# gcorso/DiffDock

Hardware: NVIDIA H100
Metric: poses/sec at 20 diffusion steps (higher is better)
Workload: dtype f32

## Files before the change

### diffdock_b200/cg_model.py

```python
from __future__ import annotations

import math
import os

import numpy as np
import torch
from torch import nn

from . import ops
from .irreps import irreps_str, sh_irreps
from .hetero import receptor_blocks
from .layers import (AtomEncoder, GaussianSmearing, _mlp, check_confidence_widths, check_forward, confidence_head, cross_cutoff,
                     cross_graph, edge_cutoff, edge_weight, ligand_graph, score_heads)
from .synthetic import LIG_FEATURE_DIMS as lig_feature_dims, REC_RESIDUE_FEATURE_DIMS as rec_residue_feature_dims
from .tensor_layers import TensorProductConvLayer, get_irrep_seq
from .tp_table import full_tensor_product

_TABLES = os.path.join(os.path.dirname(os.path.abspath(__file__)), 'tables', 'score_norm_tables.npz')
SO3_MIN_EPS, SO3_MAX_EPS, SO3_N_EPS = 0.0005, 4, 2000
TORUS_SIGMA_MIN, TORUS_SIGMA_MAX, TORUS_SIGMA_N = 3e-3, 2, 5000


def _i32(t):
    return t.to(torch.int32).contiguous()


def _flat(w):
    return w.reshape(-1).contiguous() if torch.is_tensor(w) else None


def _rr_joint(c, n_lig):
    if n_lig not in c.setdefault('rr_tgt32', {}):
        c['rr_tgt32'][n_lig] = (_i32(c['rr_tgt'] + n_lig), _i32(c['rr_src'] + n_lig))
    return c['rr_tgt32'][n_lig]


def receptor_tiles(rec, B, ei):
    blocks = receptor_blocks(rec, B, ei.shape[1])
    if blocks is None:
        return None
    dev = ei.device
    ar = lambda a, b: torch.arange(a, b, device=dev)
# ... 51 lines not shown
        self.scale_by_sigma, self.norm_by_sigma = scale_by_sigma, norm_by_sigma
        self.no_torsion, self.smooth_edges, self.odd_parity = no_torsion, smooth_edges, odd_parity
        self.confidence_mode, self.affinity_prediction = confidence_mode, affinity_prediction
        self.atom_confidence, self.atom_num_confidence_outputs = atom_confidence, atom_num_confidence_outputs
        self.num_conv_layers, self.num_prot_emb_layers = num_conv_layers, num_prot_emb_layers
        self.fixed_center_conv, self.no_aminoacid_identities = fixed_center_conv, no_aminoacid_identities
        self.differentiate_convolutions, self.reduce_pseudoscalars = differentiate_convolutions, reduce_pseudoscalars
        self.embed_also_ligand = embed_also_ligand
        self.lm_embedding_type = lm_embedding_type
        lm_dim = 1280 if lm_embedding_type == 'precomputed' else 0
        S, D, Dx = sigma_embed_dim, distance_embed_dim, cross_distance_embed_dim

        self.lig_node_embedding = AtomEncoder(emb_dim=ns, feature_dims=lig_feature_dims, sigma_embed_dim=S)
        self.lig_edge_embedding = _mlp(in_lig_edge_features + S + D, ns, ns, dropout)
        self.rec_node_embedding = AtomEncoder(emb_dim=ns, feature_dims=rec_residue_feature_dims, sigma_embed_dim=0,
                                              lm_embedding_dim=lm_dim)
        self.rec_edge_embedding = _mlp(D, ns, ns, dropout)
        self.rec_sigma_embedding = _mlp(S, ns, ns, dropout)
        self.cross_edge_embedding = _mlp(S + Dx, ns, ns, dropout)
        self.lig_distance_expansion = GaussianSmearing(0.0, lig_max_radius, D)
        self.rec_distance_expansion = GaussianSmearing(0.0, rec_max_radius, D)
        self.cross_distance_expansion = GaussianSmearing(0.0, cross_max_distance, Dx)

        self._irrep_seq = get_irrep_seq(ns, nv, use_second_order_repr, reduce_pseudoscalars)
        self._conv_kw = dict(sh_irreps=self.sh_irreps, n_edge_features=3 * ns, hidden_features=3 * ns, residual=True,
                             batch_norm=batch_norm, dropout=dropout, faster=sh_lmax == 1 and not use_second_order_repr,
                             tp_weights_layers=tp_weights_layers)
        self.rec_emb_layers = nn.ModuleList([self.conv(i, 1) for i in range(num_prot_emb_layers)])
        if embed_also_ligand:
            self.lig_emb_layers = nn.ModuleList([self.conv(i, 1) for i in range(num_prot_emb_layers)])
        self.conv_layers = self._interaction_stack(4, 2)
        self._sync_free = None
        self._prune_receptor = True
        if confidence_mode:
            self._confidence_heads(confidence_dropout, confidence_no_batchnorm, num_confidence_outputs)
            return

        self.center_distance_expansion = GaussianSmearing(0.0, center_max_distance, D)
        self.center_edge_embedding = _mlp(D + S, ns, ns, dropout)
        self.final_conv = TensorProductConvLayer(in_irreps=self.conv_layers[-1].out_irreps, sh_irreps=self.sh_irreps,
                                                 out_irreps='2x1o + 2x1e' if not odd_parity else '1x1o + 1x1e',
                                                 n_edge_features=2 * ns, residual=False, dropout=dropout,
                                                 batch_norm=batch_norm)
        self.tr_final_layer = nn.Sequential(nn.Linear(1 + S, ns), nn.Dropout(dropout), nn.ReLU(), nn.Linear(ns, 1))
        self.rot_final_layer = nn.Sequential(nn.Linear(1 + S, ns), nn.Dropout(dropout), nn.ReLU(), nn.Linear(ns, 1))
        if not no_torsion:
            self.final_edge_embedding = _mlp(D, ns, ns, dropout)
            T, tor_sh = full_tensor_product(self.sh_irreps, '1x2e')
            self.register_buffer('_tor_tp', torch.from_numpy(T).float(), persistent=False)
            self.tor_bond_conv = TensorProductConvLayer(in_irreps=self.conv_layers[-1].out_irreps,
                                                        sh_irreps=irreps_str(tor_sh),
                                                        out_irreps=f'{ns}x0o + {ns}x0e' if not odd_parity else f'{ns}x0o',
                                                        n_edge_features=3 * ns, residual=False, dropout=dropout,
                                                        batch_norm=batch_norm)
            self.tor_final_layer = nn.Sequential(nn.Linear(2 * ns if not odd_parity else ns, ns, bias=False), nn.Tanh(),
                                                 nn.Dropout(dropout), nn.Linear(ns, 1, bias=False))
        z = np.load(_TABLES)
        self.register_buffer('_so3_table', torch.from_numpy(z['so3_exp_score_norms']).float(), persistent=False)
        self.register_buffer('_torus_table', torch.from_numpy(z['torus_score_norm']).float(), persistent=False)

    def _confidence_heads(self, dropout, no_batchnorm, num_confidence_outputs):
        ns = self.ns
        self._conf_tail = (self.nv if self.reduce_pseudoscalars else ns) \
            if self.num_conv_layers + self.num_prot_emb_layers >= 3 else 0
        n_in = ns + self._conf_tail

# ... 78 lines not shown
        c['rr_ew'] = ew[order].contiguous() if torch.is_tensor(ew) else None
        c['rr_tgt_batch'] = rec.batch[tgt]
        c['rec_ptr'] = ops.segment_ptr(rec.batch, B)
        c['lig_ptr'] = ops.segment_ptr(lig.batch, B)
        mask = lig.edge_mask
        bonds = ll.edge_index[:, mask].long()
        c['bonds'], c['n_bonds'] = bonds, int(bonds.shape[1])
        c['bond_batch'] = lig.batch[bonds[0]] if bonds.shape[1] else None
        self._static_sync_free(data, c)
        rr._b200 = c
        return c

    def _static_sync_free(self, data, c):
        rec, lig, ll = data['receptor'], data['ligand'], data['ligand', 'ligand']
        B, dev = data.num_graphs, lig.pos.device
        n_lig, n_rec = lig.batch.shape[0], rec.batch.shape[0]
        lig_cnt = (c['lig_ptr'][1:] - c['lig_ptr'][:-1])
        rec_cnt = (c['rec_ptr'][1:] - c['rec_ptr'][:-1])
        host = torch.stack([lig_cnt, rec_cnt]).cpu()
        c['lig_cnt_f'] = lig_cnt.float().unsqueeze(1)
        c['rec_max'] = int(host[1].max()) if B else 0
        c['cap_cross'] = int((host[0].long() * host[1].long()).sum())
        c['lig_batch32'], c['rec_batch32'] = _i32(lig.batch), _i32(rec.batch)
        c['rr_gid32'] = _i32(c['rr_tgt_batch'])
        ei = ll.edge_index.long()
        order = torch.sort(ei[0], stable=True).indices
        c['pre_tgt'], c['pre_col'] = _i32(ei[0][order]), _i32(ei[1][order])
        attr = ll.edge_attr.float()[order] if ei.shape[1] else torch.zeros((0, self.in_lig_edge_features), device=dev)
        c['pre_attr'] = torch.cat([attr, torch.zeros((1, attr.shape[1]), device=dev)], 0)
        c['cap_ll'] = int(ei.shape[1]) + 33 * n_lig
        c['bond_lig_batch'] = lig.batch[c['bonds'][0]] if c['n_bonds'] else None
        c['cap_tor'] = 32 * c['n_bonds']
        c['bond_batch32'] = _i32(c['bond_batch']) if c['n_bonds'] else None

    def _ligand_graph(self, data, c):
        tgt, src, attr, vec, ew, node = ligand_graph(self, data, c['lig_ptr'])
        tgt, order = torch.sort(tgt, stable=True)
        return node, tgt, src[order], attr[order], vec[order], ew[order] if torch.is_tensor(ew) else ew

    def sync_free_capable(self):
        if self._sync_free is None:
            ok = os.environ.get('DDB200_SYNC_FREE', '1') != '0'
            ok = ok and self.embed_also_ligand
            for layer in list(self.conv_layers) + list(getattr(self, 'lig_emb_layers', [])):
                ok = ok and layer.fused_capable(self.ns, self.ns)
            self._sync_free = bool(ok)
        return self._sync_free

    def sync_free_crop_capable(self):
        return self.sync_free_capable() and all(layer.fused_capable(self.ns, self.ns) for layer in self.rec_emb_layers)

    @torch.no_grad()
    def forward(self, data):
        check_forward(self, data)
        c = self._static(data)
        if self.sync_free_capable() and max(c['rec_max'], c.get('atom_max', 0)) <= 10000:
            return self._forward_sync_free(data, c)
        if getattr(data, '_crop', None) is not None:
            raise RuntimeError("per-step receptor cropping (data._crop) runs on the sync-free forward only, which this "
                               "batch cannot take (more than 10000 residues in a complex)")
        return self._forward_host_sized(data, c)

    def _interaction_layers(self, node, groups, n_last, merge=False, shared=None, per_layer=None):
        L = len(self.conv_layers)
        for l, layer in enumerate(self.conv_layers):
            use, init = (groups if l < L - 1 else groups[:n_last]), None
# ... 1 lines not shown
                k = per_layer[0]
                use = use[:k] + [per_layer[1][l]] + use[k + 1:]
            if l == 0 and shared is not None:
                init, skip = shared
                use = use[:skip] + [None] + use[skip + 1:]
            if merge:
                use = [tuple(torch.cat([g[k] for g in use]) if use[0][k] is not None else None for k in range(5))]
            node = layer.forward_groups(node, use, gather_scalars=self.ns, init=init)
        return node

    def _forward_sync_free(self, data, c):
        lig, rec = data['ligand'], data['receptor']
        ns, n_lig = self.ns, lig.batch.shape[0]
        tr_sigma, rot_sigma, tor_sigma = self._sigmas(data)

        sig = self.rec_sigma_embedding(self.timestep_emb_func(data.complex_t['tr'])).contiguous()
        crop = getattr(data, '_crop', None)
        prune = self._prune_receptor and len(self.conv_layers) > 1
        keep = None
        if crop is None:
            rec_node, rec_pos = rec.rec_node_attr.clone(), rec.pos.float().contiguous()
            rr_tgt32 = _rr_joint(c, n_lig)
            g_rr = (rr_tgt32[0], rr_tgt32[1], c['rr_ea'], c['rr_vec'], _flat(c['rr_ew']),
                    dict(ea_add=sig, ea_add_idx=c['rr_gid32']))
        else:
            rec_node, rec_pos, g_rr, keep = self._cropped_receptor(data, c, crop, sig, n_lig, select=not prune)
        rec_node[:, :ns] += sig[rec.batch]
        lig_node, g_ll = self._ligand_graph_sync_free(data, c)

        r, rpg = cross_cutoff(self, tr_sigma)
        g_lr, g_rl = self._cross_graph_sync_free(data, c, rec_pos, c['rec_ptr'], c['rec_batch32'],
                                                 c['rec_max'], c['cap_cross'], r, rpg, n_lig, self.cross_edge_embedding,
                                                 self.cross_distance_expansion, vec_sign=-1.0)

        node = torch.cat([lig_node, rec_node], 0)
        groups = [g_ll,
                  g_lr,
                  g_rr,
                  g_rl]
        shared = self._shared_receptor_messages(data, c, rec, rec_node, sig, n_lig) \
            if len(self.conv_layers) > 1 and crop is None else None
        pruned = self._pruned_contact_groups(c, g_rl, keep, sig, n_lig, rec_node.shape[0], shared is not None) \
            if prune else None
        node = self._interaction_layers(node, groups, 2, shared=(shared, 2) if shared is not None else None,
                                        per_layer=(2, pruned) if pruned is not None else None)
        return self._heads(data, c, node[:n_lig], tr_sigma, rot_sigma, tor_sigma, sync_free=True)

    def _need_levels(self, L, shared):
        return [None if l == L - 1 or (l == 0 and shared) else L - 1 - l for l in range(L)]

    def _pruned_contact_groups(self, c, g_rl, keep, sig, n_lig, n_rec, shared):
        levels = self._need_levels(len(self.conv_layers), shared)
        n_levels = max((k for k in levels if k is not None), default=0)
        if n_levels == 0:
            return None
        if 'rr_tgt32l' not in c:
            c['rr_tgt32l'] = (_i32(c['rr_tgt']), _i32(c['rr_src']))
        tgt32, src32 = c['rr_tgt32l']
        key = ('prune', n_lig, n_levels)
        if key not in c:
            c[key] = (torch.empty((n_levels, n_rec), dtype=torch.uint8, device=tgt32.device),
                      [ops.select_edges_buffers(tgt32.shape[0], tgt32.device) for _ in range(n_levels)])
        need_buf, bufs = c[key]
        need = ops.receptor_need(g_rl[0], g_rl[5]['n_edges_dev'], n_lig, tgt32, src32, n_rec, n_levels, keep=keep,
                                 out=need_buf)
        ew, sel = _flat(c['rr_ew']), {}
# ... 175 lines not shown
```

### diffdock_b200/csrc/fused_conv.cu

```cuda
#include <cuda_bf16.h>
#include <cuda_runtime.h>
#include <stdint.h>
#include <stdlib.h>

#include "../../include/diffdock_b200.h"
#include "sm90.cuh"

namespace {

using namespace ddb200_sm90;

constexpr int BM = 64, BK = 64;
constexpr int CTA_EDGES = 2 * BM;
constexpr int A_KB_BYTES = BM * BK * 2;
constexpr int B_IMAGE_BYTES = 256 * BK * 2;
constexpr int MAX_N = 192;
constexpr int STAGES = 4;
constexpr int STAGE_BYTES = MAX_N * BK * 2;
constexpr int MAX_KB = 5;
constexpr int MAX_KA = MAX_KB;
constexpr int A_IMAGE_BYTES = MAX_KA * A_KB_BYTES;
constexpr int OPS_PER_KB = 8;
constexpr int THREADS = 256;
constexpr int MAX_TILES = 128, MAX_PATHS = 16, MTAB = 48;
// ... 702 lines not shown
struct DeviceState {
  bool attr_done = false, attr_done_so = false;
  bool dbg_init = false;
  unsigned long long* dbg = nullptr;
};
DeviceState g_dev[MAX_DEVICES];

unsigned long long* fused_debug_buffer(int dev) {
  if (dev < 0 || dev >= MAX_DEVICES) return nullptr;
  DeviceState& st = g_dev[dev];
  if (!st.dbg_init) {
    st.dbg_init = true;
    const char* e = getenv("DDB200_FUSED_DEBUG");
    if (e && atoi(e) != 0 && cudaMalloc(&st.dbg, 32 * sizeof(unsigned long long)) == cudaSuccess)
      cudaMemset(st.dbg, 0, 32 * sizeof(unsigned long long));
  }
  return st.dbg;
}

}


extern "C" int ddb200_fused_debug_read(uint64_t* out) {
  int dev = 0;
  cudaGetDevice(&dev);
  unsigned long long* b = fused_debug_buffer(dev);
  if (!b || !out) return DDB200_EINVAL;
  cudaError_t e = cudaDeviceSynchronize();
  if (e == cudaSuccess) e = cudaMemcpy(out, b, 32 * sizeof(unsigned long long), cudaMemcpyDeviceToHost);
  if (e == cudaSuccess) e = cudaMemset(b, 0, 32 * sizeof(unsigned long long));
  return (int)e;
}

namespace {

template <bool SO>
int fused_conv_launch(const ddb200_fused_args* a, void* stream) {
  if (!a || !a->edge_attr || !a->w1_images || !a->w2_images || !a->tiles || !a->mtab || !a->x || !a->edge_vec || !a->sum ||
      !a->tgt || !a->src || a->n_edges < 0 || a->ne <= 0 || a->ns < 0 || a->hidden <= 0 || a->n_tiles <= 0 || a->d_out <= 0)
    return DDB200_EINVAL;
  if (a->ns > 0 && (!a->node || a->ld_node < a->ns)) return DDB200_EINVAL;
  if (a->n_tiles > MAX_TILES || a->n_paths <= 0 || a->n_paths > (SO ? SO_MAX_PATHS : MAX_PATHS) || a->sh_lmax < 0 ||
      a->sh_lmax > 2)
    return DDB200_EINVAL;
  if ((a->ea_add == nullptr) != (a->ea_add_idx == nullptr)) return DDB200_EINVAL;
  const int K1 = a->ne + 2 * a->ns, H = a->hidden;
  const int K1p = (K1 + 15) / 16 * 16, Hp = (H + 15) / 16 * 16;
  const int n_kb = (2 * Hp + 16 + BK - 1) / BK, n_kb1 = (2 * K1p + 16 + BK - 1) / BK;
  if (n_kb > MAX_KB || n_kb1 > MAX_KB || H > MAX_N) return DDB200_EINVAL;
  if ((reinterpret_cast<uintptr_t>(a->w1_images) & 127) || (reinterpret_cast<uintptr_t>(a->w2_images) & 127)) return DDB200_EINVAL;
  if (a->n_hidden < 0 || (a->n_hidden > 0 && (!a->wh_images || (reinterpret_cast<uintptr_t>(a->wh_images) & 127))))
    return DDB200_EINVAL;
  if (a->n_edges == 0) return 0;
  FusedParams p = {};
  p.ea = a->edge_attr; p.ld_ea = a->ld_ea; p.ne = a->ne; p.node = a->node; p.ld_node = a->ld_node; p.ns = a->ns;
  p.tgt = a->tgt; p.src = a->src; p.perm = a->edge_perm; p.ea_add = a->ea_add; p.ea_add_idx = a->ea_add_idx;
  const auto al16 = [](const void* q) { return (reinterpret_cast<uintptr_t>(q) & 15) == 0; };
  p.a0_vec = ((a->ne | a->ns) & 7) == 0 && ((a->ld_ea | (a->ns ? a->ld_node : 0)) & 3) == 0 && al16(a->edge_attr) &&
             (a->ns == 0 || al16(a->node)) && (a->ea_add == nullptr || al16(a->ea_add));
  p.vec_sign = a->vec_sign == 0.f ? 1.f : a->vec_sign;
  p.w1img = reinterpret_cast<const __nv_bfloat16*>(a->w1_images); p.K1 = K1; p.K1p = K1p; p.n_kb1 = n_kb1;
  p.H = H; p.Hp = Hp; p.n_kb = n_kb;
  p.w2img = reinterpret_cast<const __nv_bfloat16*>(a->w2_images); p.tiles = a->tiles; p.n_tiles = a->n_tiles;
  p.whimg = reinterpret_cast<const __nv_bfloat16*>(a->wh_images); p.n_hidden = a->n_hidden;
  p.mtab = a->mtab; p.n_paths = a->n_paths;
  p.x = a->x; p.ld_x = a->ld_x; p.x_vec2 = (a->x_pairs_ok && (a->ld_x & 1) == 0 && (reinterpret_cast<uintptr_t>(a->x) & 7) == 0) ? 1 : 0;
  p.vec = a->edge_vec; p.ew = a->edge_weight; p.lmax = a->sh_lmax; p.sum = a->sum; p.d_out = a->d_out; p.cnt = a->cnt;
  p.n_edges = a->n_edges; p.n_edges_dev = a->n_edges_dev;
  int dev = 0, sms = 132;
  cudaGetDevice(&dev);
  if (dev < 0 || dev >= MAX_DEVICES) return DDB200_EINVAL;
  p.dbg = fused_debug_buffer(dev);
  cudaDeviceGetAttribute(&sms, cudaDevAttrMultiProcessorCount, dev);
  const long long n_mtiles = (a->n_edges + CTA_EDGES - 1) / CTA_EDGES;
  const size_t smem = smem_bytes<SO>();
  if (smem > 227 * 1024) return DDB200_ESMEM;
  auto kernel = SO ? fused_conv_kernel_so : fused_conv_kernel;
  bool& attr_done = SO ? g_dev[dev].attr_done_so : g_dev[dev].attr_done;
  if (!attr_done) {
    const cudaError_t e = cudaFuncSetAttribute(kernel, cudaFuncAttributeMaxDynamicSharedMemorySize, (int)smem);
    if (e != cudaSuccess) return (int)e;
    attr_done = true;
  }
  const unsigned grid = (unsigned)(n_mtiles < sms ? n_mtiles : sms);
  kernel<<<grid, THREADS, smem, (cudaStream_t)stream>>>(p);
  return (int)cudaGetLastError();
}

}

extern "C" int ddb200_fused_conv(const ddb200_fused_args* a, void* stream) { return fused_conv_launch<false>(a, stream); }

extern "C" int ddb200_fused_conv_so(const ddb200_fused_args* a, void* stream) { return fused_conv_launch<true>(a, stream); }
```

### diffdock_b200/fused.py

```python
from __future__ import annotations

import ctypes as C
import os

import numpy as np
import torch

from . import _lib
from .ops import PROFILE, _need_cuda, _ptr, _stream

from .irreps import real_cg
from .radial import BK, BN
from .tp_table import TpTable

CONSUMER_KINDS = {(48, 1): (0, 4), (10, 3): (1, 16), (16, 1): (2, 8), (4, 3): (3, 16), (10, 1): (4, 16), (4, 1): (5, 16),
                  (10, 5): (6, 16), (4, 5): (7, 16)}
MAX_K = 144
MAX_TILES = 128
MTAB = 48
MAX_PATHS = 16
MTAB_SO = 128
MAX_PATHS_SO = 32
ENABLED = os.environ.get('DDB200_FUSED_CONV', '1') != '0'


def _pad16(k: int) -> int:
    return (k + 15) // 16 * 16


def second_order(table: TpTable) -> bool:
    return any(p.l_in == 2 or p.l_out == 2 for p in table.paths)


def supported(table: TpTable, hidden: int, k1: int) -> bool:
    if table.sh_lmax < 0 or table.sh_lmax > 2:
        return False
    if _pad16(hidden) > MAX_K or _pad16(k1) > MAX_K:
        return False
    if len(table.paths) > (MAX_PATHS_SO if second_order(table) else MAX_PATHS):
        return False
    for p in table.paths:
        if (p.mul_out, 2 * p.l_out + 1) not in CONSUMER_KINDS:
            return False
        if (2 * p.l_in + 1) not in (1, 3, 5) or p.l_sh > 2:
            return False
    n_tiles = sum(-(-p.mul_in // CONSUMER_KINDS[(p.mul_out, 2 * p.l_out + 1)][1]) for p in table.paths)
    return n_tiles <= MAX_TILES


def _split_images(w_rows: torch.Tensor, bias_rows: torch.Tensor, K: int):
    T = w_rows.shape[0]
    Kp = _pad16(K)
    n_kb = (2 * Kp + 16 + BK - 1) // BK
    dev = w_rows.device
    hi = w_rows.to(torch.bfloat16)
# ... 49 lines not shown
                src[:nrow * p.mul_out] = cols
                row_src.append(src)
        for i in range(len(tiles)):
            if i == len(tiles) - 1 or tiles[i + 1][6] & 1:
                tiles[i][6] |= 2
        self.n_tiles = len(tiles)
        self.n_paths = len(paths)
        src = torch.as_tensor(np.stack(row_src), device=dev)
        ok = src >= 0
        w_rows = torch.zeros((self.n_tiles, BN, H), dtype=torch.float32, device=dev)
        b_rows = torch.zeros((self.n_tiles, BN), dtype=torch.float32, device=dev)
        w_rows[ok] = w2_ref.detach().float()[src[ok]]
        b_rows[ok] = b2_ref.detach().float()[src[ok]]
        self.w2_images = _split_images(w_rows, b_rows, H)
        w1p = torch.zeros((1, BN, K1), dtype=torch.float32, device=dev)
        b1p = torch.zeros((1, BN), dtype=torch.float32, device=dev)
        w1p[0, :H], b1p[0, :H] = w1.detach().float(), b1.detach().float()
        self.w1_images = _split_images(w1p, b1p, K1)
        self.wh_images = None
        if hidden:
            whp = torch.zeros((self.n_hidden, BN, H), dtype=torch.float32, device=dev)
            bhp = torch.zeros((self.n_hidden, BN), dtype=torch.float32, device=dev)
            for l, (w, b) in enumerate(hidden):
                whp[l, :H], bhp[l, :H] = w.detach().float(), b.detach().float()
            self.wh_images = _split_images(whp, bhp, H)
        self.tiles = torch.as_tensor(np.asarray(tiles, dtype=np.int32), device=dev).contiguous()
        self.mtab = torch.as_tensor(mtab, device=dev).contiguous()
        self.x_pairs_ok = int(all(t[2] % 2 == 0 and (t[3] * t[4]) % 2 == 0 for t in tiles))
        s2, s1 = 3 * (_pad16(H) // 16) + 1, 3 * (_pad16(K1) // 16) + 1
        self.mma_flops_per_tile = 2 * 64 * 16 * 192 * (s1 + (self.n_hidden + len(tiles)) * s2)
        self.alg_flops_per_edge = 2 * K1 * H + self.n_hidden * 2 * H * H + 2 * H * table.weight_numel + sum(
            2 * p.mul_in * p.mul_out * (2 * p.l_out + 1) + 2 * p.mul_in * (2 * p.l_in + 1) * (2 * p.l_sh + 1) * (2 * p.l_out + 1)
            for p in table.paths)


class _Args(C.Structure):
    _fields_ = [('edge_attr', C.c_void_p), ('ld_ea', C.c_int64), ('ne', C.c_int32),
                ('node', C.c_void_p), ('ld_node', C.c_int64), ('ns', C.c_int32),
                ('tgt', C.c_void_p), ('src', C.c_void_p), ('edge_perm', C.c_void_p),
                ('ea_add', C.c_void_p), ('ea_add_idx', C.c_void_p), ('vec_sign', C.c_float),
                ('w1_images', C.c_void_p), ('hidden', C.c_int32), ('w2_images', C.c_void_p),
                ('tiles', C.c_void_p), ('n_tiles', C.c_int32), ('mtab', C.c_void_p), ('n_paths', C.c_int32),
                ('x', C.c_void_p), ('ld_x', C.c_int64), ('x_pairs_ok', C.c_int32),
                ('edge_vec', C.c_void_p), ('edge_weight', C.c_void_p), ('sh_lmax', C.c_int32),
                ('n_edges', C.c_int64), ('n_edges_dev', C.c_void_p),
                ('sum', C.c_void_p), ('d_out', C.c_int32), ('cnt', C.c_void_p),
                ('wh_images', C.c_void_p), ('n_hidden', C.c_int32)]


def _p(t):
    return t.data_ptr() if t is not None else None


def fused_conv(plan: FusedPlan, edge_attr, node, ns, tgt32, src32, x, edge_vec, sum_buf, cnt_buf, edge_weight=None,
               edge_perm=None, vec_sign=1.0, ea_add=None, ea_add_idx=None, n_edges_dev=None, n_edges=None):
    _need_cuda(edge_attr, x, edge_vec, sum_buf)
    ne = edge_attr.shape[1]
    E = int(tgt32.shape[0]) if n_edges is None else int(n_edges)
    if E == 0:
        return
    t = plan.table
    assert edge_attr.dtype == torch.float32 and edge_attr.stride(1) == 1 and x.stride(1) == 1 and edge_vec.is_contiguous()
    assert edge_vec.dtype == torch.float32 and x.dtype == torch.float32 and sum_buf.dtype == torch.float32
    assert tgt32.dtype == torch.int32 and src32.dtype == torch.int32 and tgt32.is_contiguous() and src32.is_contiguous()
    assert ne + 2 * ns == plan.k1 and x.shape[1] == t.d_in and sum_buf.shape[1] == t.d_out and sum_buf.is_contiguous()
    if edge_perm is None:
        assert edge_attr.shape[0] >= E and edge_vec.shape[0] >= E
    else:
        assert edge_perm.dtype == torch.int32 and edge_perm.is_contiguous() and edge_perm.shape[0] >= E
    if edge_weight is not None:
        edge_weight = edge_weight.reshape(-1)
        assert edge_weight.dtype == torch.float32 and edge_weight.is_contiguous()
    if ea_add is not None:
        assert ea_add.dtype == torch.float32 and ea_add.is_contiguous() and ea_add.shape[1] == ne
        assert ea_add_idx.dtype == torch.int32 and ea_add_idx.is_contiguous() and ea_add_idx.shape[0] >= E
    if n_edges_dev is not None:
        assert n_edges_dev.dtype == torch.int32 and n_edges_dev.is_cuda
    a = _Args(_p(edge_attr), edge_attr.stride(0), ne, _p(node) if ns else None, node.stride(0) if ns else 0, ns,
              _p(tgt32), _p(src32), _p(edge_perm), _p(ea_add), _p(ea_add_idx) if ea_add is not None else None,
              float(vec_sign), _p(plan.w1_images), plan.hidden, _p(plan.w2_images), _p(plan.tiles), plan.n_tiles,
              _p(plan.mtab), plan.n_paths, _p(x), x.stride(0), plan.x_pairs_ok, _p(edge_vec), _p(edge_weight),
              t.sh_lmax, E, _p(n_edges_dev), _p(sum_buf), t.d_out, _p(cnt_buf), _p(plan.wh_images), plan.n_hidden)
    prof = PROFILE.enabled
    if prof:
        e0, e1 = torch.cuda.Event(enable_timing=True), torch.cuda.Event(enable_timing=True)
        e0.record()
    launch = _lib.lib().ddb200_fused_conv_so if plan.second_order else _lib.lib().ddb200_fused_conv
    rc = launch(C.byref(a), _stream())
    if prof:
        e1.record()
        n_live = int(n_edges_dev.item()) if n_edges_dev is not None else E
        PROFILE.fused_pairs.append((e0, e1))
        PROFILE.fused_bytes += n_live * (4 * t.weight_numel + 12 + 4) + 4 * (sum_buf.shape[0] + 1) + \
            4 * x.shape[0] * t.d_in + 4 * sum_buf.shape[0] * t.d_out
        PROFILE.fused_flops += ((n_live + 63) // 64) * plan.mma_flops_per_tile
        PROFILE.fused_alg_flops += n_live * plan.alg_flops_per_edge
    PROFILE.all_launches += 1
    _lib.check(rc, 'ddb200_fused_conv')
```

### include/diffdock_b200.h

```cpp
#ifndef DIFFDOCK_B200_H
#define DIFFDOCK_B200_H

#include <stddef.h>
#include <stdint.h>

#ifdef __cplusplus
extern "C" {
#endif

#define DDB200_EINVAL (-1)
#define DDB200_ETABLE (-2)
#define DDB200_ESMEM  (-3)

const char* ddb200_version(void);

typedef struct ddb200_tp_table ddb200_tp_table;

int  ddb200_tp_table_create(const int32_t* iblob_host, int n_ints, const float* fblob_host, int n_floats,
                            ddb200_tp_table** out);
void ddb200_tp_table_destroy(ddb200_tp_table* t);
int  ddb200_tp_table_info(const ddb200_tp_table* t, int what);

int ddb200_tpconv_accumulate(const ddb200_tp_table* t, const float* x, int64_t x_stride, const int32_t* edge_src,
                             const int32_t* edge_dst, const float* geo, const float* edge_weight, const float* w,
// ... 36 lines not shown

int ddb200_csr_sort_by_target(const int32_t* tgt, int64_t n_edges, int32_t n_rows, int32_t* tgt_sorted, int32_t* perm,
                              int32_t* row_ptr, void* workspace, size_t* workspace_bytes, void* stream);

int ddb200_edge_embed(const float* edge_vec, const int32_t* edge_row, const float* u, const float* w1_rbf, const float* w2,
                      const float* b2, int rbf_dim, int ns, const float* rbf_offset, float rbf_coeff, int64_t capacity,
                      const int32_t* n_edges_dev, float* out, void* stream);

int ddb200_radial_gemm(const float* h, int64_t ldh, int64_t n_edges, int K, const void* b_images, const float* bias,
                       int n_tiles_n, float* out, int64_t ldo, void* stream);

int ddb200_radial_mlp(const float* edge_attr, int64_t ld_ea, int ne, const float* node, int64_t ld_node, int ns,
                      const int32_t* tgt, const int32_t* src, const void* w1_images, const float* b1, int hidden,
                      const void* w2_images, const float* b2, int n_tiles_n, int64_t n_edges, float* out, int64_t ldo,
                      void* stream);

typedef struct ddb200_fused_args {
  const float*   edge_attr;   int64_t ld_ea;   int32_t ne;
  const float*   node;        int64_t ld_node; int32_t ns;
  const int32_t* tgt;         const int32_t* src;
  const int32_t* edge_perm;
  const float*   ea_add;      const int32_t* ea_add_idx;
  float          vec_sign;
  const void*    w1_images;   int32_t hidden;
  const void*    w2_images;
  const int32_t* tiles;       int32_t n_tiles;
  const float*   mtab;        int32_t n_paths;
  const float*   x;           int64_t ld_x;    int32_t x_pairs_ok;
  const float*   edge_vec;    const float* edge_weight;
  int32_t        sh_lmax;
  int64_t        n_edges;     const int32_t* n_edges_dev;
  float*         sum;         int32_t d_out;   float* cnt;
  const void*    wh_images;   int32_t n_hidden;
} ddb200_fused_args;

int ddb200_fused_conv(const ddb200_fused_args* args, void* stream);
int ddb200_fused_conv_so(const ddb200_fused_args* args, void* stream);

int ddb200_fused_debug_read(uint64_t* out);

int ddb200_contact_count(const float* pos, int32_t n, float cutoff, int32_t max_neighbors, int32_t knn_only,
                         int32_t* count, void* stream);
int ddb200_contact_fill(const float* pos, int32_t n, float cutoff, int32_t max_neighbors, int32_t knn_only,
                        const int32_t* row_start, int32_t* out_nbr, int32_t* out_ctr, void* stream);

int ddb200_crop_flags(const float* lig_pos, const int32_t* lig_ptr, const float* rec_pos, const int32_t* rec_batch,
                      int64_t n_rec, const float* cutoff2_table, const int32_t* step_dev, uint8_t* keep,
                      float* rec_pos_masked, void* stream);
int ddb200_crop_select_edges(const int32_t* tgt, const int32_t* src, const int32_t* gid, int64_t n_edges,
                             const uint8_t* keep, const uint8_t* need, int32_t offset, int32_t* out_tgt, int32_t* out_src,
                             int32_t* out_perm, int32_t* out_gid, int32_t* n_selected, void* workspace,
                             size_t* workspace_bytes, void* stream);
int ddb200_receptor_need(const int32_t* cross_tgt, const int32_t* n_cross, int64_t cross_cap, int32_t offset,
                         const int32_t* tgt, const int32_t* src, int64_t n_edges, const uint8_t* keep, int64_t n_rec,
                         int32_t n_levels, uint8_t* need, void* stream);

#define DDB200_CONF_MAX_IN 256
#define DDB200_CONF_MAX_HIDDEN 128
#define DDB200_CONF_MAX_OUT 16
int ddb200_confidence_head(const float* x, int64_t ld_x, int64_t n_cols, const int32_t* lig_ptr, int32_t n_poses,
                           int32_t n_head, int32_t tail_off, int32_t n_tail, const float* atom_mlp, int32_t atom_hidden,
                           int32_t n_atom_out, const float* mlp, int32_t n_in, int32_t n_hidden, int32_t n_out,
                           float* confidence, float* atom_confidence, void* stream);

#ifdef __cplusplus
}
// ... 3 lines not shown
```

Baseline: 23.78.

## Add per-target reassociated tensor-product sum for dense ligand-receptor cross edges

```diff
diff --git a/diffdock_b200/cg_model.py b/diffdock_b200/cg_model.py
--- a/diffdock_b200/cg_model.py
+++ b/diffdock_b200/cg_model.py
@@ -7,7 +7,7 @@
 import torch
 from torch import nn
 
-from . import ops
+from . import fused, ops
 from .irreps import irreps_str, sh_irreps
 from .hetero import receptor_blocks
 from .layers import (AtomEncoder, GaussianSmearing, _mlp, check_confidence_widths, check_forward, confidence_head, cross_cutoff,
@@ -125,6 +125,7 @@
         self.conv_layers = self._interaction_stack(4, 2)
         self._sync_free = None
         self._prune_receptor = True
+        self._ligand_target_sum = True
         if confidence_mode:
             self._confidence_heads(confidence_dropout, confidence_no_batchnorm, num_confidence_outputs)
             return
@@ -269,6 +270,24 @@
         c['bond_lig_batch'] = lig.batch[c['bonds'][0]] if c['n_bonds'] else None
         c['cap_tor'] = 32 * c['n_bonds']
         c['bond_batch32'] = _i32(c['bond_batch']) if c['n_bonds'] else None
+        if getattr(self, '_ligand_target_sum', False):
+            c['lr_target_sum'] = self._ligand_target_sum_workspace(c['cap_cross'], n_lig, dev)
+
+    def _ligand_receptor_plans(self):
+        plans = []
+        for layer in self.conv_layers:
+            fc = layer.fc if layer.edge_groups == 1 else list(layer.fc)[1]
+            plans.append(layer._fused_plan(fc, layer.tp.table_vec, 3 * self.ns) if layer.tp.vec_capable else None)
+        return plans
+
+    def _ligand_target_sum_workspace(self, cap_cross, n_lig, dev):
+        if not (type(self)._forward_sync_free is CGModel._forward_sync_free and not self.confidence_mode
+                and self.sync_free_capable() and cap_cross > 0):
+            return None
+        plans = self._ligand_receptor_plans()
+        if any(p is None or not p.per_target_ok for p in plans):
+            return None
+        return fused.TargetSumWorkspace(cap_cross, n_lig, plans[0].hidden, max(p.ts_zp for p in plans), dev)
 
     def _ligand_graph(self, data, c):
         tgt, src, attr, vec, ew, node = ligand_graph(self, data, c['lig_ptr'])
@@ -336,6 +355,11 @@
         g_lr, g_rl = self._cross_graph_sync_free(data, c, rec_pos, c['rec_ptr'], c['rec_batch32'],
                                                  c['rec_max'], c['cap_cross'], r, rpg, n_lig, self.cross_edge_embedding,
                                                  self.cross_distance_expansion, vec_sign=-1.0)
+        if self._ligand_target_sum:
+            if 'lr_target_sum' not in c:
+                c['lr_target_sum'] = self._ligand_target_sum_workspace(c['cap_cross'], n_lig, lig.pos.device)
+            if c['lr_target_sum'] is not None:
+                g_lr[5]['per_target'] = c['lr_target_sum']
 
         node = torch.cat([lig_node, rec_node], 0)
         groups = [g_ll,
diff --git a/diffdock_b200/csrc/fused_conv.cu b/diffdock_b200/csrc/fused_conv.cu
--- a/diffdock_b200/csrc/fused_conv.cu
+++ b/diffdock_b200/csrc/fused_conv.cu
@@ -758,6 +758,8 @@
   return (int)e;
 }
 
+int target_sum_launch(const ddb200_fused_args* a, void* stream);
+
 namespace {
 
 template <bool SO>
@@ -777,7 +779,12 @@
   if ((reinterpret_cast<uintptr_t>(a->w1_images) & 127) || (reinterpret_cast<uintptr_t>(a->w2_images) & 127)) return DDB200_EINVAL;
   if (a->n_hidden < 0 || (a->n_hidden > 0 && (!a->wh_images || (reinterpret_cast<uintptr_t>(a->wh_images) & 127))))
     return DDB200_EINVAL;
+  if (a->per_target && SO) return DDB200_EINVAL;
   if (a->n_edges == 0) return 0;
+  if (a->per_target) {
+    const int rc = target_sum_launch(a, stream);
+    if (rc) return rc;
+  }
   FusedParams p = {};
   p.ea = a->edge_attr; p.ld_ea = a->ld_ea; p.ne = a->ne; p.node = a->node; p.ld_node = a->ld_node; p.ns = a->ns;
   p.tgt = a->tgt; p.src = a->src; p.perm = a->edge_perm; p.ea_add = a->ea_add; p.ea_add_idx = a->ea_add_idx;
@@ -792,7 +799,7 @@
   p.mtab = a->mtab; p.n_paths = a->n_paths;
   p.x = a->x; p.ld_x = a->ld_x; p.x_vec2 = (a->x_pairs_ok && (a->ld_x & 1) == 0 && (reinterpret_cast<uintptr_t>(a->x) & 7) == 0) ? 1 : 0;
   p.vec = a->edge_vec; p.ew = a->edge_weight; p.lmax = a->sh_lmax; p.sum = a->sum; p.d_out = a->d_out; p.cnt = a->cnt;
-  p.n_edges = a->n_edges; p.n_edges_dev = a->n_edges_dev;
+  p.n_edges = a->n_edges; p.n_edges_dev = a->per_target ? a->ts_sel + 1 : a->n_edges_dev;
   int dev = 0, sms = 132;
   cudaGetDevice(&dev);
   if (dev < 0 || dev >= MAX_DEVICES) return DDB200_EINVAL;
diff --git a/diffdock_b200/csrc/target_sum.cu b/diffdock_b200/csrc/target_sum.cu
--- /dev/null
+++ b/diffdock_b200/csrc/target_sum.cu
@@ -0,0 +1,344 @@
+#include <cuda_runtime.h>
+#include <stdint.h>
+
+#include "../../include/diffdock_b200.h"
+
+namespace {
+
+constexpr int TS_THREADS = 256;
+constexpr int HP = 144;
+constexpr int A_THREADS = 512, A_EDGES = 128, A_LD = A_EDGES + 4;
+constexpr int ZC = 128, CE = 32, HR = 160;
+constexpr int C_TARGETS = 4, C_JSPLIT = 29;
+
+struct TsParams {
+  const float* ea; long long ld_ea; int ne;
+  const float* node; long long ld_node; int ns;
+  const int* tgt; const int* src; const int* perm;
+  const float* ea_add; const int* ea_add_idx;
+  float vec_sign;
+  const float* x; long long ld_x;
+  const float* vec; const float* ew;
+  const float* mtab;
+  float* sum; int d_out; float* cnt;
+  long long n_edges; const int* n_edges_dev;
+  int K1, H;
+  float* hid; int ld;
+  float* S; long long n_targets; int zp;
+  const float* w1t; const float* b1; const float* w2bt; int w2_ld;
+  const int* cols; const int* paths; const int* items; int n_items;
+  int* sel; long long min_edges;
+};
+
+__device__ __forceinline__ long long live_edges(const TsParams& p) {
+  long long n = p.n_edges;
+  if (p.n_edges_dev) { const long long nd = __ldg(p.n_edges_dev); n = nd < n ? (nd < 0 ? 0 : nd) : n; }
+  return n;
+}
+
+__device__ __forceinline__ long long lower_bound(const int* tgt, long long n, int a) {
+  long long lo = 0, hi = n;
+  while (lo < hi) {
+    const long long mid = (lo + hi) >> 1;
+    if (__ldg(tgt + mid) < a) lo = mid + 1; else hi = mid;
+  }
+  return lo;
+}
+
+__device__ __forceinline__ void red_add(float* addr, float v) {
+  asm volatile("red.global.add.f32 [%0], %1;" ::"l"(addr), "f"(v) : "memory");
+}
+
+__global__ void target_sum_select_kernel(const TsParams p) {
+  const long long n = live_edges(p);
+  const int on = n >= p.min_edges;
+  p.sel[0] = on;
+  p.sel[1] = on ? 0 : (int)n;
+}
+
+__global__ void __launch_bounds__(A_THREADS) target_sum_hidden_kernel(const TsParams p) {
+  extern __shared__ __align__(16) float smem[];
+  if (!__ldg(p.sel)) return;
+  float* w1t = smem;
+  float* b1 = w1t + p.K1 * HP;
+  float* aT = b1 + HP;
+  const int tid = threadIdx.x;
+  for (int i = tid; i < p.K1 * HP; i += A_THREADS) w1t[i] = __ldg(p.w1t + i);
+  for (int i = tid; i < HP; i += A_THREADS) b1[i] = __ldg(p.b1 + i);
+  const long long n = live_edges(p);
+  const int eg = tid >> 4, hg = tid & 15;
+  for (long long e0 = (long long)blockIdx.x * A_EDGES; e0 < n; e0 += (long long)gridDim.x * A_EDGES) {
+    __syncthreads();
+    for (int i = tid; i < A_EDGES * p.K1; i += A_THREADS) {
+      const int r = i / p.K1, k = i - r * p.K1;
+      const long long e = e0 + r;
+      float v = 0.f;
+      if (e < n) {
+        if (k < p.ne) {
+          const long long er = p.perm ? (long long)__ldg(p.perm + e) : e;
+          v = __ldg(p.ea + er * p.ld_ea + k);
+          if (p.ea_add) v += __ldg(p.ea_add + (long long)__ldg(p.ea_add_idx + e) * p.ne + k);
+        } else if (k < p.ne + p.ns) v = __ldg(p.node + (long long)__ldg(p.tgt + e) * p.ld_node + (k - p.ne));
+        else v = __ldg(p.node + (long long)__ldg(p.src + e) * p.ld_node + (k - p.ne - p.ns));
+      }
+      aT[k * A_LD + r] = v;
+    }
+    __syncthreads();
+    float acc[4][9];
+#pragma unroll
+    for (int i = 0; i < 4; ++i)
+#pragma unroll
+      for (int j = 0; j < 9; ++j) acc[i][j] = 0.f;
+#pragma unroll 2
+    for (int k = 0; k < p.K1; ++k) {
+      const float4 a = *reinterpret_cast<const float4*>(aT + k * A_LD + 4 * eg);
+      const float* w = w1t + k * HP + hg;
+#pragma unroll
+      for (int j = 0; j < 9; ++j) {
+        const float wv = w[16 * j];
+        acc[0][j] = fmaf(a.x, wv, acc[0][j]);
+        acc[1][j] = fmaf(a.y, wv, acc[1][j]);
+        acc[2][j] = fmaf(a.z, wv, acc[2][j]);
+        acc[3][j] = fmaf(a.w, wv, acc[3][j]);
+      }
+    }
+#pragma unroll
+    for (int i = 0; i < 4; ++i) {
+      const long long e = e0 + 4 * eg + i;
+      if (e >= n) continue;
+      const long long er = p.perm ? (long long)__ldg(p.perm + e) : e;
+      const float ew = p.ew ? __ldg(p.ew + er) : 1.f;
+      float* row = p.hid + e * p.ld;
+#pragma unroll
+      for (int j = 0; j < 9; ++j) {
+        const int c = hg + 16 * j;
+        if (c < p.H) row[c] = ew * fmaxf(acc[i][j] + b1[c], 0.f);
+      }
+      if (hg < p.ld - p.H) row[p.H + hg] = hg == 0 ? ew : 0.f;
+    }
+  }
+}
+
+__global__ void __launch_bounds__(TS_THREADS, 2) target_sum_accumulate_kernel(const TsParams p) {
+  __shared__ __align__(16) float hs[CE * HR];
+  __shared__ __align__(16) float zs[CE * ZC];
+  __shared__ float ys[CE * 9];
+  __shared__ float mks[15 * ZC];
+  __shared__ int ss[CE];
+  const int tid = threadIdx.x, a = blockIdx.y;
+  if (!__ldg(p.sel)) return;
+  const long long n = live_edges(p);
+  const long long lo = lower_bound(p.tgt, n, a), hi = lower_bound(p.tgt, n, a + 1);
+  if (lo >= hi) return;
+  const int c = tid & (ZC - 1), col = blockIdx.x * ZC + c;
+  const int4 cd = __ldg(reinterpret_cast<const int4*>(p.cols) + col);
+  const int path = cd.x, xoff = cd.y, d_in = cd.z, kk = cd.w & 0xff, sh = (cd.w >> 8) & 0xff;
+  if (tid < ZC)
+    for (int ij = 0; ij < 15; ++ij) {
+      const int i = ij / 5, j = ij - 5 * i;
+      mks[ij * ZC + c] = (path >= 0 && i < d_in) ? __ldg(p.mtab + path * 48 + (i * 3 + kk) * 5 + j) : 0.f;
+    }
+  for (int i = tid; i < CE * HR; i += TS_THREADS)
+    if ((i % HR) >= p.ld) hs[i] = 0.f;
+  const int rg = tid >> 4, cg = tid & 15;
+  float acc[10][8];
+#pragma unroll
+  for (int r = 0; r < 10; ++r)
+#pragma unroll
+    for (int q = 0; q < 8; ++q) acc[r][q] = 0.f;
+  const int nq = p.ld >> 2;
+  for (long long c0 = lo; c0 < hi; c0 += CE) {
+    const int m = (int)min((long long)CE, hi - c0);
+    __syncthreads();
+    for (int i = tid; i < CE * nq; i += TS_THREADS) {
+      const int e = i / nq, q4 = i - e * nq;
+      float4 v = make_float4(0.f, 0.f, 0.f, 0.f);
+      if (e < m) v = __ldg(reinterpret_cast<const float4*>(p.hid + (c0 + e) * p.ld) + q4);
+      *reinterpret_cast<float4*>(hs + e * HR + 4 * q4) = v;
+    }
+    if (tid < CE) {
+      const long long e = c0 + tid;
+      float* Y = ys + tid * 9;
+      if (tid < m) {
+        const long long er = p.perm ? (long long)__ldg(p.perm + e) : e;
+        float vx = p.vec_sign * __ldg(p.vec + 3 * er), vy = p.vec_sign * __ldg(p.vec + 3 * er + 1),
+              vz = p.vec_sign * __ldg(p.vec + 3 * er + 2);
+        const float nrm = fmaxf(sqrtf(vx * vx + vy * vy + vz * vz), 1e-12f);
+        vx /= nrm; vy /= nrm; vz /= nrm;
+        const float s3 = 1.7320508075688772f, s5 = 2.23606797749979f, s15 = 3.872983346207417f;
+        Y[0] = 1.f;
+        Y[1] = s3 * vx; Y[2] = s3 * vy; Y[3] = s3 * vz;
+        Y[4] = s15 * vx * vz;
+        Y[5] = s15 * vx * vy;
+        Y[6] = s5 * (vy * vy - 0.5f * (vx * vx + vz * vz));
+        Y[7] = s15 * vy * vz;
+        Y[8] = 0.5f * s15 * (vz * vz - vx * vx);
+        ss[tid] = __ldg(p.src + e);
+      } else {
+        ss[tid] = -1;
+      }
+    }
+    __syncthreads();
+#pragma unroll 2
+    for (int e = tid / ZC; e < CE; e += TS_THREADS / ZC) {
+      float z = 0.f;
+      const int s = ss[e];
+      if (s >= 0 && path >= 0) {
+        const float* xr = p.x + (long long)s * p.ld_x + xoff;
+        const float* Y = ys + e * 9;
+        float yb[5];
+#pragma unroll
+        for (int j = 0; j < 5; ++j) yb[j] = Y[min(sh + j, 8)];
+#pragma unroll
+        for (int i = 0; i < 3; ++i) {
+          if (i < d_in) {
+            float mi = 0.f;
+#pragma unroll
+            for (int j = 0; j < 5; ++j) mi = fmaf(mks[(i * 5 + j) * ZC + c], yb[j], mi);
+            z = fmaf(__ldg(xr + i), mi, z);
+          }
+        }
+      }
+      zs[e * ZC + c] = z;
+    }
+    __syncthreads();
+    for (int e = 0; e < m; ++e) {
+      const float4 z0 = *reinterpret_cast<const float4*>(zs + e * ZC + 4 * cg);
+      const float4 z1 = *reinterpret_cast<const float4*>(zs + e * ZC + 64 + 4 * cg);
+      const float zv[8] = {z0.x, z0.y, z0.z, z0.w, z1.x, z1.y, z1.z, z1.w};
+      const float2* hp = reinterpret_cast<const float2*>(hs + e * HR + 10 * rg);
+#pragma unroll
+      for (int r2 = 0; r2 < 5; ++r2) {
+        const float2 h = hp[r2];
+#pragma unroll
+        for (int q = 0; q < 8; ++q) {
+          acc[2 * r2][q] = fmaf(h.x, zv[q], acc[2 * r2][q]);
+          acc[2 * r2 + 1][q] = fmaf(h.y, zv[q], acc[2 * r2 + 1][q]);
+        }
+      }
+    }
+  }
+  float* Sa = p.S + (long long)a * (p.H + 1) * p.zp + blockIdx.x * ZC + 4 * cg;
+#pragma unroll
+  for (int r = 0; r < 10; ++r) {
+    const int j = 10 * rg + r;
+    if (j <= p.H) {
+      *reinterpret_cast<float4*>(Sa + (long long)j * p.zp) = make_float4(acc[r][0], acc[r][1], acc[r][2], acc[r][3]);
+      *reinterpret_cast<float4*>(Sa + (long long)j * p.zp + 64) = make_float4(acc[r][4], acc[r][5], acc[r][6], acc[r][7]);
+    }
+  }
+}
+
+template <int D>
+__device__ __forceinline__ void output_item(const TsParams& p, const float* const* Sa, const bool* live, int pi, int w0,
+                                            int j0, int j1, int a0) {
+  const int* P = p.paths + pi * 8;
+  const int zoff = __ldg(P), mul_in = __ldg(P + 1), mul_out = __ldg(P + 2), out_off = __ldg(P + 4), wref = __ldg(P + 5);
+  float acc[C_TARGETS][2][D];
+#pragma unroll
+  for (int t = 0; t < C_TARGETS; ++t)
+#pragma unroll
+    for (int w = 0; w < 2; ++w)
+#pragma unroll
+      for (int k = 0; k < D; ++k) acc[t][w][k] = 0.f;
+  for (int u = 0; u < mul_in; ++u) {
+    const int row = wref + u * mul_out + w0, zc = zoff + u * D;
+    for (int j = j0; j < j1; ++j) {
+      const float2 wv = __ldg(reinterpret_cast<const float2*>(p.w2bt + (long long)j * p.w2_ld + row));
+#pragma unroll
+      for (int t = 0; t < C_TARGETS; ++t) {
+        const float* s = Sa[t] + (long long)j * p.zp + zc;
+#pragma unroll
+        for (int k = 0; k < D; ++k) {
+          const float sv = __ldg(s + k);
+          acc[t][0][k] = fmaf(wv.x, sv, acc[t][0][k]);
+          acc[t][1][k] = fmaf(wv.y, sv, acc[t][1][k]);
+        }
+      }
+    }
+  }
+#pragma unroll
+  for (int t = 0; t < C_TARGETS; ++t) {
+    if (!live[t]) continue;
+    float* o = p.sum + (long long)(a0 + t) * p.d_out + out_off + w0 * D;
+#pragma unroll
+    for (int w = 0; w < 2; ++w)
+#pragma unroll
+      for (int k = 0; k < D; ++k) red_add(o + w * D + k, acc[t][w][k]);
+  }
+}
+
+__global__ void __launch_bounds__(TS_THREADS) target_sum_output_kernel(const TsParams p) {
+  __shared__ bool live[C_TARGETS];
+  __shared__ const float* Sa[C_TARGETS];
+  const int tid = threadIdx.x, a0 = blockIdx.x * C_TARGETS;
+  if (!__ldg(p.sel)) return;
+  if (tid < C_TARGETS) {
+    const int a = a0 + tid;
+    bool l = false;
+    if (a < p.n_targets) {
+      const long long n = live_edges(p);
+      const long long cnt = lower_bound(p.tgt, n, a + 1) - lower_bound(p.tgt, n, a);
+      l = cnt > 0;
+      if (l && p.cnt && blockIdx.y == 0) red_add(p.cnt + a, (float)cnt);
+    }
+    live[tid] = l;
+    Sa[tid] = p.S + (long long)(l ? a : a0) * (p.H + 1) * p.zp;
+  }
+  __syncthreads();
+  bool any = false;
+#pragma unroll
+  for (int t = 0; t < C_TARGETS; ++t) any |= live[t];
+  if (!any) return;
+  const int per = (p.H + 1 + C_JSPLIT - 1) / C_JSPLIT, j0 = blockIdx.y * per, j1 = min(p.H + 1, j0 + per);
+  for (int it = tid; it < p.n_items; it += blockDim.x) {
+    const int pi = __ldg(p.items + 2 * it), w0 = __ldg(p.items + 2 * it + 1);
+    if (__ldg(p.paths + pi * 8 + 3) == 1) output_item<1>(p, Sa, live, pi, w0, j0, j1, a0);
+    else output_item<3>(p, Sa, live, pi, w0, j0, j1, a0);
+  }
+}
+
+bool g_attr_done[64];
+
+}
+
+int target_sum_launch(const ddb200_fused_args* a, void* stream) {
+  const int K1 = a->ne + 2 * a->ns, H = a->hidden;
+  if (a->n_hidden != 0 || K1 > HP || H > HP || !a->ts_hidden || !a->ts_s || !a->ts_w1t || !a->ts_b1 || !a->ts_w2bt ||
+      !a->ts_cols || !a->ts_paths || !a->ts_items || !a->ts_sel || a->ts_n_items <= 0 || a->ts_targets <= 0 || a->ts_zp <= 0 ||
+      a->ts_zp % ZC || a->ts_ld < H + 1 || a->ts_ld % 4 || a->ts_ld > HR || a->ts_w2_ld % 2 ||
+      (reinterpret_cast<uintptr_t>(a->ts_hidden) & 15) || (reinterpret_cast<uintptr_t>(a->ts_s) & 15) ||
+      (reinterpret_cast<uintptr_t>(a->ts_w2bt) & 7) || (reinterpret_cast<uintptr_t>(a->ts_cols) & 15))
+    return DDB200_EINVAL;
+  if (a->ts_targets > 65535) return DDB200_EINVAL;
+  if (a->n_edges == 0) return 0;
+  TsParams p = {};
+  p.ea = a->edge_attr; p.ld_ea = a->ld_ea; p.ne = a->ne; p.node = a->node; p.ld_node = a->ld_node; p.ns = a->ns;
+  p.tgt = a->tgt; p.src = a->src; p.perm = a->edge_perm; p.ea_add = a->ea_add; p.ea_add_idx = a->ea_add_idx;
+  p.vec_sign = a->vec_sign == 0.f ? 1.f : a->vec_sign;
+  p.x = a->x; p.ld_x = a->ld_x; p.vec = a->edge_vec; p.ew = a->edge_weight; p.mtab = a->mtab;
+  p.sum = a->sum; p.d_out = a->d_out; p.cnt = a->cnt; p.n_edges = a->n_edges; p.n_edges_dev = a->n_edges_dev;
+  p.K1 = K1; p.H = H; p.hid = a->ts_hidden; p.ld = a->ts_ld; p.S = a->ts_s; p.n_targets = a->ts_targets; p.zp = a->ts_zp;
+  p.w1t = a->ts_w1t; p.b1 = a->ts_b1; p.w2bt = a->ts_w2bt; p.w2_ld = a->ts_w2_ld;
+  p.cols = a->ts_cols; p.paths = a->ts_paths; p.items = a->ts_items; p.n_items = a->ts_n_items;
+  p.sel = a->ts_sel; p.min_edges = a->ts_min_edges;
+  int dev = 0, sms = 132;
+  cudaGetDevice(&dev);
+  if (dev < 0 || dev >= 64) return DDB200_EINVAL;
+  cudaDeviceGetAttribute(&sms, cudaDevAttrMultiProcessorCount, dev);
+  const size_t smem_a = ((size_t)K1 * HP + HP + (size_t)K1 * A_LD) * sizeof(float);
+  const unsigned c_threads = (unsigned)min(TS_THREADS, (a->ts_n_items + 31) / 32 * 32);
+  if (!g_attr_done[dev]) {
+    const cudaError_t e = cudaFuncSetAttribute(target_sum_hidden_kernel, cudaFuncAttributeMaxDynamicSharedMemorySize,
+                                               (int)((size_t)HP * HP + HP + (size_t)HP * A_LD) * (int)sizeof(float));
+    if (e != cudaSuccess) return (int)e;
+    g_attr_done[dev] = true;
+  }
+  cudaStream_t s = (cudaStream_t)stream;
+  const long long tiles = (a->n_edges + A_EDGES - 1) / A_EDGES;
+  target_sum_select_kernel<<<1, 1, 0, s>>>(p);
+  target_sum_hidden_kernel<<<(unsigned)(tiles < sms ? tiles : sms), A_THREADS, smem_a, s>>>(p);
+  target_sum_accumulate_kernel<<<dim3((unsigned)(a->ts_zp / ZC), (unsigned)a->ts_targets), TS_THREADS, 0, s>>>(p);
+  target_sum_output_kernel<<<dim3((unsigned)((a->ts_targets + C_TARGETS - 1) / C_TARGETS), C_JSPLIT), c_threads, 0, s>>>(p);
+  return (int)cudaGetLastError();
+}
diff --git a/diffdock_b200/fused.py b/diffdock_b200/fused.py
--- a/diffdock_b200/fused.py
+++ b/diffdock_b200/fused.py
@@ -21,6 +21,8 @@
 MAX_PATHS = 16
 MTAB_SO = 128
 MAX_PATHS_SO = 32
+TS_ZC = 128
+TS_MIN_EDGES_PER_TARGET = 700
 ENABLED = os.environ.get('DDB200_FUSED_CONV', '1') != '0'
 
 
@@ -136,6 +138,53 @@
         self.alg_flops_per_edge = 2 * K1 * H + self.n_hidden * 2 * H * H + 2 * H * table.weight_numel + sum(
             2 * p.mul_in * p.mul_out * (2 * p.l_out + 1) + 2 * p.mul_in * (2 * p.l_in + 1) * (2 * p.l_sh + 1) * (2 * p.l_out + 1)
             for p in table.paths)
+        self.per_target_ok = not self.second_order and self.n_hidden == 0
+        if self.per_target_ok:
+            self._target_sum_tables(paths, mtab.shape[1], w1, b1, w2_ref, b2_ref)
+
+    def _target_sum_tables(self, paths, mtab_ld, w1, b1, w2_ref, b2_ref):
+        dev, H, K1 = w2_ref.device, self.hidden, self.k1
+        z_off, cols, prow = 0, [], []
+        for pi, p in enumerate(paths):
+            d_in, d_out = 2 * p.l_in + 1, 2 * p.l_out + 1
+            assert p.mul_out % 2 == 0 and p.w_ref_off % 2 == 0
+            for u in range(p.mul_in):
+                for k in range(d_out):
+                    cols.append([pi, p.in_off + u * d_in, d_in, k | (p.sh_off << 8)])
+            prow.append([z_off, p.mul_in, p.mul_out, d_out, p.out_off, p.w_ref_off, 0, 0])
+            z_off += p.mul_in * d_out
+        self.ts_z = z_off
+        self.ts_zp = -(-z_off // TS_ZC) * TS_ZC
+        cols += [[-1, 0, 1, 0]] * (self.ts_zp - z_off)
+        self.ts_cols = torch.as_tensor(np.asarray(cols, dtype=np.int32), device=dev).contiguous()
+        self.ts_paths = torch.as_tensor(np.asarray(prow, dtype=np.int32), device=dev).contiguous()
+        items = [[pi, w0] for pi, p in enumerate(paths) for w0 in range(0, p.mul_out, 2)]
+        self.ts_items = torch.as_tensor(np.asarray(items, dtype=np.int32), device=dev).contiguous()
+        self.ts_w1t = torch.zeros((K1, MAX_K), dtype=torch.float32, device=dev)
+        self.ts_w1t[:, :H] = w1.detach().float().T
+        self.ts_b1 = torch.zeros(MAX_K, dtype=torch.float32, device=dev)
+        self.ts_b1[:H] = b1.detach().float()
+        W = self.table.weight_numel
+        self.ts_w2_ld = W + (W & 1)
+        self.ts_w2bt = torch.zeros((H + 1, self.ts_w2_ld), dtype=torch.float32, device=dev)
+        self.ts_w2bt[:H, :W] = w2_ref.detach().float().T
+        self.ts_w2bt[H, :W] = b2_ref.detach().float()
+        self.ts_ld = -(-(H + 1) // 4) * 4
+
+
+class TargetSumWorkspace:
+
+    def __init__(self, edge_capacity, n_targets, hidden, zp, device, min_edges=None):
+        self.n_targets, self.hidden_units, self.zp = int(n_targets), int(hidden), int(zp)
+        self.min_edges = int(min_edges) if min_edges is not None else TS_MIN_EDGES_PER_TARGET * self.n_targets
+        self.sel = torch.zeros(2, dtype=torch.int32, device=device)
+        self.ld = -(-(hidden + 1) // 4) * 4
+        self.hidden = torch.empty((max(int(edge_capacity), 1), self.ld), dtype=torch.float32, device=device)
+        self.s = torch.empty((max(self.n_targets, 1) * (hidden + 1) * self.zp,), dtype=torch.float32, device=device)
+
+    @staticmethod
+    def nbytes(edge_capacity, n_targets, hidden, zp):
+        return 4 * (edge_capacity * (-(-(hidden + 1) // 4) * 4) + n_targets * (hidden + 1) * zp)
 
 
 class _Args(C.Structure):
@@ -149,7 +198,12 @@
                 ('edge_vec', C.c_void_p), ('edge_weight', C.c_void_p), ('sh_lmax', C.c_int32),
                 ('n_edges', C.c_int64), ('n_edges_dev', C.c_void_p),
                 ('sum', C.c_void_p), ('d_out', C.c_int32), ('cnt', C.c_void_p),
-                ('wh_images', C.c_void_p), ('n_hidden', C.c_int32)]
+                ('wh_images', C.c_void_p), ('n_hidden', C.c_int32),
+                ('per_target', C.c_int32), ('ts_hidden', C.c_void_p), ('ts_ld', C.c_int32),
+                ('ts_s', C.c_void_p), ('ts_targets', C.c_int64), ('ts_zp', C.c_int32),
+                ('ts_w1t', C.c_void_p), ('ts_b1', C.c_void_p), ('ts_w2bt', C.c_void_p), ('ts_w2_ld', C.c_int32),
+                ('ts_cols', C.c_void_p), ('ts_paths', C.c_void_p), ('ts_items', C.c_void_p), ('ts_n_items', C.c_int32),
+                ('ts_sel', C.c_void_p), ('ts_min_edges', C.c_int64)]
 
 
 def _p(t):
@@ -157,7 +211,7 @@
 
 
 def fused_conv(plan: FusedPlan, edge_attr, node, ns, tgt32, src32, x, edge_vec, sum_buf, cnt_buf, edge_weight=None,
-               edge_perm=None, vec_sign=1.0, ea_add=None, ea_add_idx=None, n_edges_dev=None, n_edges=None):
+               edge_perm=None, vec_sign=1.0, ea_add=None, ea_add_idx=None, n_edges_dev=None, n_edges=None, per_target=None):
     _need_cuda(edge_attr, x, edge_vec, sum_buf)
     ne = edge_attr.shape[1]
     E = int(tgt32.shape[0]) if n_edges is None else int(n_edges)
@@ -185,6 +239,15 @@
               float(vec_sign), _p(plan.w1_images), plan.hidden, _p(plan.w2_images), _p(plan.tiles), plan.n_tiles,
               _p(plan.mtab), plan.n_paths, _p(x), x.stride(0), plan.x_pairs_ok, _p(edge_vec), _p(edge_weight),
               t.sh_lmax, E, _p(n_edges_dev), _p(sum_buf), t.d_out, _p(cnt_buf), _p(plan.wh_images), plan.n_hidden)
+    if per_target is not None:
+        ws = per_target
+        assert plan.per_target_ok and ws.hidden_units == plan.hidden and ws.zp >= plan.ts_zp and ws.hidden.shape[0] >= E
+        a.per_target, a.ts_hidden, a.ts_ld = 1, _p(ws.hidden), ws.ld
+        a.ts_s, a.ts_targets, a.ts_zp = _p(ws.s), ws.n_targets, plan.ts_zp
+        a.ts_w1t, a.ts_b1, a.ts_w2bt, a.ts_w2_ld = _p(plan.ts_w1t), _p(plan.ts_b1), _p(plan.ts_w2bt), plan.ts_w2_ld
+        a.ts_cols, a.ts_paths, a.ts_items, a.ts_n_items = (_p(plan.ts_cols), _p(plan.ts_paths), _p(plan.ts_items),
+                                                           int(plan.ts_items.shape[0]))
+        a.ts_sel, a.ts_min_edges = _p(ws.sel), ws.min_edges
     prof = PROFILE.enabled
     if prof:
         e0, e1 = torch.cuda.Event(enable_timing=True), torch.cuda.Event(enable_timing=True)
diff --git a/include/diffdock_b200.h b/include/diffdock_b200.h
--- a/include/diffdock_b200.h
+++ b/include/diffdock_b200.h
@@ -92,6 +92,12 @@
   int64_t        n_edges;     const int32_t* n_edges_dev;
   float*         sum;         int32_t d_out;   float* cnt;
   const void*    wh_images;   int32_t n_hidden;
+  int32_t        per_target;
+  float*         ts_hidden;   int32_t ts_ld;
+  float*         ts_s;        int64_t ts_targets;   int32_t ts_zp;
+  const float*   ts_w1t;      const float* ts_b1;   const float* ts_w2bt;   int32_t ts_w2_ld;
+  const int32_t* ts_cols;     const int32_t* ts_paths;   const int32_t* ts_items;   int32_t ts_n_items;
+  int32_t*       ts_sel;      int64_t ts_min_edges;
 } ddb200_fused_args;
 
 int ddb200_fused_conv(const ddb200_fused_args* args, void* stream);
```

New measurement: 23.98 (median of 6 runs). About the same (+0.9%).
